# Yuming-Yang/FactorModeling

Measured on AMD Instinct MI355X. Metric: factor·asset·days/s (ops+IC+select), higher is better.
Workload: dtype f64

## Files before the change

factormodeling_amd/csrc/rank_ic.hip:

```cpp
#include "rank_fine.hpp"
#include "rank_launch.hpp"

namespace fmx {

__global__ void k_ic_empty(double* out, int64_t F, int64_t D, int L0, int L1, int NL) {
  const int64_t f = blockIdx.x;
  for (int m = 0; m < NL; ++m) {
    const int L = m == 0 ? L0 : L1;
    for (int64_t td = threadIdx.x; td < min<int64_t>(L, D); td += blockDim.x) {
      double* o = out + ((int64_t)(m * 4) * F + f) * D + td;
      o[0] = 0.0;
      o[F * D] = qnan();
      o[2 * F * D] = qnan();
      o[3 * F * D] = qnan();
    }
  }
}


fmx_status br_ic_daily(const double* X, const double* R, int64_t F, int64_t D, int64_t A, int64_t ld,
                       const int32_t* lags_host, int n_lags, double* out, hipStream_t st) {
  const int nt = A <= 4096 ? 512 : 1024;
  const size_t lds_fr = std::max<size_t>((size_t)(FRG<FR_K_IC>::NB + 1) * 8, (size_t)A * 13 + 16);
  auto fr_table = FMX_EMAX_TABLE(k_ic_daily_fr);
  const bool fine = rank_impl() == RANK_IMPL_FINE && lds_fits(fr_table(nt, br_emax(A, nt)), lds_fr);
  const size_t lds = fine ? lds_fr : (size_t)std::max<int64_t>(A, nt) * 8 + (size_t)((A + 15) & ~15ll);
  if (!fine && !lds_fits(FMX_EMAX_TABLE(k_ic_daily_br)(nt, br_emax(A, nt)), lds)) {
    set_error("row too long for the IC kernels' LDS (rank it once with fmx_cs_rank_winsor and use "
              "fmx_ic_daily_ranked)");
    return FMX_ERR_UNSUPPORTED;
  }
  for (int base = 0; base < n_lags; base += 2) {
    int NL = std::min(2, n_lags - base);
    int L0 = lags_host[base], L1 = NL > 1 ? lags_host[base + 1] : 0;
    double* o = out + (int64_t)base * 4 * F * D;
    k_ic_empty<<<(unsigned)F, 64, 0, st>>>(o, F, D, L0, L1, NL);
    FMX_LAUNCH_CHECK("k_ic_empty");
    void* args[] = {(void*)&X, (void*)&R, (void*)&F, (void*)&D, (void*)&A, (void*)&ld, (void*)&L0, (void*)&L1,
                    (void*)&NL, (void*)&o};
    fmx_status e = fine ? launch_br(fr_table, nt, A, F, D, lds, args, st)
                        : launch_br(FMX_EMAX_TABLE(k_ic_daily_br), nt, A, F, D, lds, args, st);
    if (e) return e;
  }
  return FMX_OK;
}

constexpr int ICW_PC = 256;
__global__ void __launch_bounds__(256)
k_nan_positions(const double* __restrict__ Rt, int64_t D, int64_t A, int64_t ld, int32_t* __restrict__ pos,
                int32_t* __restrict__ npos) {
  const int lane = threadIdx.x & 63;
  const int64_t d = (int64_t)blockIdx.x * 4 + (threadIdx.x >> 6);
  if (d >= D) return;
  const double* r = Rt + d * ld;
  const uint64_t lt = (1ull << lane) - 1ull;
  int c = 0;
  for (int64_t i0 = 0; i0 < A; i0 += 64) {
    const int64_t i = i0 + lane;
    const bool nan = i < A && !(r[i] == r[i]);
    const uint64_t b = __ballot(nan);
    const int at = c + __popcll(b & lt);
    if (nan && at < ICW_PC) pos[d * ICW_PC + at] = (int32_t)i;
    c += __popcll(b);
  }
  if (lane == 0) npos[d] = c;
}

constexpr int ICW_WAVES = 4;
#ifndef ICW_PF
#define ICW_PF 1
#endif
constexpr int ICW_EC = 256;
constexpr uint64_t ICW_NO_ENTRY = 0xffffffff00000000ull;

#ifndef ICW_MINW
#define ICW_MINW 6
#endif
__global__ void __launch_bounds__(64 * ICW_WAVES, ICW_MINW)
k_ic_wave(const double* __restrict__ X, const fmx_rank2_t* __restrict__ RK, const double* __restrict__ Rt, int64_t F,
          int64_t D, int64_t A, int64_t ld, int L0, int L1, int NL, double* __restrict__ out,
          const int32_t* __restrict__ pos, const int32_t* __restrict__ npos, int32_t* __restrict__ ovf) {
  extern __shared__ uint32_t icw_lds[];
  __shared__ double scr[ICW_WAVES * 32];
  const int lane = threadIdx.x & 63, wid = __builtin_amdgcn_readfirstlane((int)(threadIdx.x >> 6));
  const int64_t row = (int64_t)blockIdx.x * ICW_WAVES + wid;
  if (row >= F * D) return;
  const int64_t s = row / F, f = row % F;
  const int lagv[2] = {L0, L1};
  const double* rr[2];
  bool act[2];
#pragma unroll
  for (int m = 0; m < 2; ++m) {
    act[m] = m < NL && s + lagv[m] < D;
    rr[m] = Rt + (act[m] ? s + lagv[m] : s) * ld;
  }
  if (!act[0] && !act[1]) return;
  const double* xf = X + (f * D + s) * ld;
  const fmx_rank2_t* rkf = RK + (f * D + s) * ld;
  const int nb = (int)((2 * A) >> 6) + 1;
  const int nbp = (nb + 1) & ~1;
  uint32_t* T[2];
  uint64_t* T64[2];
  uint32_t* eb[2];
#pragma unroll
  for (int m = 0; m < 2; ++m) {
    T[m] = icw_lds + (wid * 2 + m) * (2 * nbp + ICW_EC);
    T64[m] = reinterpret_cast<uint64_t*>(T[m]);
    eb[m] = T[m] + 2 * nbp;
  }
  int ne[2] = {0, 0};
  bool over = false;
  uint32_t er[2][ICW_EC / 64];
  int es[2][ICW_EC / 64];
  const int An = (int)A;
  double xq[ICW_PF], rq[ICW_PF][2];
  uint32_t kq[ICW_PF];
  auto load = [&](int i0, int s) {
    const int i = i0 + lane;
    if (i0 + 64 <= An) {
      xq[s] = xf[i];
      kq[s] = (uint32_t)rkf[i];
#pragma unroll
      for (int m = 0; m < 2; ++m) rq[s][m] = rr[m][i];
    } else {
      const bool in = i < An;
      xq[s] = in ? xf[i] : qnan();
      kq[s] = in ? (uint32_t)rkf[i] : 0u;
#pragma unroll
      for (int m = 0; m < 2; ++m) rq[s][m] = in ? rr[m][i] : qnan();
    }
  };
#pragma unroll
  for (int s = 0; s < ICW_PF; ++s) load(64 * s, s);
#pragma unroll
  for (int m = 0; m < 2; ++m) {
    for (int b = lane; b < nbp; b += 64) T64[m][b] = 0ull;
#pragma unroll
    for (int q = 0; q < ICW_EC / 64; ++q) { er[m][q] = 0u; es[m][q] = 0; }
  }
  __builtin_amdgcn_wave_barrier();
  int cl[2];
#pragma unroll
  for (int m = 0; m < 2; ++m) cl[m] = act[m] ? npos[s + lagv[m]] : 0;
  over = cl[0] > ICW_PC || cl[1] > ICW_PC;
  if (!over) {
    const int cmax = cl[0] > cl[1] ? cl[0] : cl[1];
    const int32_t* pp[2] = {pos + (s + (act[0] ? lagv[0] : 0)) * ICW_PC, pos + (s + (act[1] ? lagv[1] : 0)) * ICW_PC};
#pragma unroll
    for (int q = 0; q < ICW_EC / 64; ++q) {
      if (64 * q >= cmax) break;
      const int j = 64 * q + lane;
      int p[2];
#pragma unroll
      for (int m = 0; m < 2; ++m) p[m] = pp[m][j];
#pragma unroll
      for (int m = 0; m < 2; ++m) p[m] = j < cl[m] ? p[m] : 0;
      uint32_t r2[2];
#pragma unroll
      for (int m = 0; m < 2; ++m) r2[m] = (uint32_t)rkf[p[m]];
#pragma unroll
      for (int m = 0; m < 2; ++m) {
        const uint32_t e = j < cl[m] ? r2[m] : 0u;
        er[m][q] = e;
        if (e) es[m][q] = (int)atomicAdd(&T[m][e >> 6], 1u);
        ne[m] += __popcll(__ballot(e != 0u));
      }
    }
  }
  if (over) {
    if (lane == 0) {
      const int q = atomicAdd(&ovf[0], 1);
      ovf[1 + q] = (int32_t)row;
    }
    return;
  }
  __builtin_amdgcn_wave_barrier();
#pragma unroll
  for (int m = 0; m < 2; ++m) {
    if (ne[m] == 0) continue;
    constexpr int RMAX = 9;
    const int R = (nbp + 63) >> 6;
    int cn[RMAX];
    int loc = 0;
#pragma unroll
    for (int q = 0; q < RMAX; ++q) {
      const int b = lane * R + q;
      cn[q] = (q < R && b < nbp) ? (int)T[m][b] : 0;
      loc += cn[q];
    }
    int incl = loc;
#pragma unroll
    for (int o = 1; o < 64; o <<= 1) {
      const int u = fr_up(incl, o, lane);
      if (lane >= o) incl += u;
    }
    int run = incl - loc;
    int st[RMAX];
    asm volatile("s_waitcnt lgkmcnt(0)" ::: "memory");
    __builtin_amdgcn_wave_barrier();
#pragma unroll
    for (int q = 0; q < RMAX; ++q) {
      const int b = lane * R + q;
      st[q] = run;
      if (q < R && b < nbp) T64[m][b] = ICW_NO_ENTRY | (uint64_t)((uint32_t)(2 * run) | ((uint32_t)cn[q] << 16));
      run += cn[q];
    }
    asm volatile("s_waitcnt lgkmcnt(0)" ::: "memory");
    __builtin_amdgcn_wave_barrier();
#pragma unroll
    for (int q = 0; q < ICW_EC / 64; ++q)
      if (er[m][q]) eb[m][(((uint32_t)T64[m][er[m][q] >> 6] & 0xffffu) >> 1) + es[m][q]] = er[m][q];
    asm volatile("s_waitcnt lgkmcnt(0)" ::: "memory");
    __builtin_amdgcn_wave_barrier();
#pragma unroll
    for (int q = 0; q < RMAX; ++q) {
      const int b = lane * R + q;
      if (q < R && b < nbp && cn[q] > 0) {
        const uint64_t e0 = eb[m][st[q]], e1 = cn[q] > 1 ? eb[m][st[q] + 1] : 0xffffu;
        T64[m][b] = (uint64_t)((uint32_t)(2 * st[q]) | ((uint32_t)cn[q] << 16)) | (e0 << 32) | (e1 << 48);
      }
    }
  }
#pragma unroll
  for (int m = 0; m < 2; ++m)
    if (ne[m] == 0)
      for (int b = lane; b < nbp; b += 64) T64[m][b] = ICW_NO_ENTRY;
  __builtin_amdgcn_wave_barrier();
  double sm[2][6];
  uint64_t kk[2] = {0, 0};
  double ax[2] = {0.0, 0.0}, ar[2] = {0.0, 0.0};
  bool ref[2] = {false, false};
  int cnt[2] = {0, 0};
  uint64_t dm[4] = {0, 0, 0, 0};
#pragma unroll
  for (int m = 0; m < 2; ++m)
#pragma unroll
    for (int q = 0; q < 6; ++q) sm[m][q] = 0.0;
  auto next = [&](int i0, double& x, uint32_t& rk, double (&r)[2]) {
    x = xq[0];
    rk = kq[0];
    r[0] = rq[0][0];
    r[1] = rq[0][1];
#pragma unroll
    for (int s = 0; s + 1 < ICW_PF; ++s) {
      xq[s] = xq[s + 1];
      kq[s] = kq[s + 1];
      rq[s][0] = rq[s + 1][0];
      rq[s][1] = rq[s + 1][1];
    }
    if (i0 + 64 * ICW_PF < An) load(i0 + 64 * ICW_PF, ICW_PF - 1);
  };
  auto pair_rank = [&](int m, uint32_t rk) {
    const uint64_t tb = T64[m][rk >> 6];
    const uint32_t lo = (uint32_t)tb, hi = (uint32_t)(tb >> 32);
    const uint32_t j0 = (lo & 0xffffu) >> 1, nj = lo >> 16, j1 = j0 + nj;
    const uint32_t e0 = hi & 0xffffu, e1 = hi >> 16;
    int corr = (int)(lo & 0xffffu) + (e0 < rk ? 1 : 0) + (e0 <= rk ? 1 : 0) + (e1 < rk ? 1 : 0) + (e1 <= rk ? 1 : 0);
    for (uint32_t j = j0 + 2; j < j1; ++j) {
      const uint32_t e = eb[m][j];
      corr += (e < rk ? 1 : 0) + (e <= rk ? 1 : 0);
    }
    return rk - (uint32_t)corr;
  };
  auto accum = [&](int m, bool p, uint64_t bp, double x, uint32_t k2, double r) {
    dm[2 * m] |= bp & __ballot(x != ax[m]);
    dm[2 * m + 1] |= bp & __ballot(r != ar[m]);
    if (!p) return;
    const double dx = x - ax[m], dy = r - ar[m];
    sm[m][0] += dx; sm[m][1] += dy;
    sm[m][2] = __builtin_fma(dx, dx, sm[m][2]);
    sm[m][3] = __builtin_fma(dy, dy, sm[m][3]);
    sm[m][4] = __builtin_fma(dx, dy, sm[m][4]);
    sm[m][5] = __builtin_fma((double)k2, dy, sm[m][5]);
    kk[m] += (uint64_t)k2 * k2;
  };
  ref[0] = !act[0];
  ref[1] = !act[1];
  int i0 = 0;
  for (; i0 < An && !(ref[0] && ref[1]); i0 += 64) {
    double x, r[2];
    uint32_t rk;
    next(i0, x, rk, r);
    const uint32_t k2[2] = {pair_rank(0, rk), pair_rank(1, rk)};
#pragma unroll
    for (int m = 0; m < 2; ++m) {
      const bool p = (x == x) & (r[m] == r[m]);
      const uint64_t bp = __ballot(p);
      cnt[m] += __popcll(bp);
      if (!ref[m] && bp) {
        const int l = __ffsll((unsigned long long)bp) - 1;
        ax[m] = fr_readlane_d(x, l);
        ar[m] = fr_readlane_d(r[m], l);
        ref[m] = true;
      }
      if (ref[m]) accum(m, p, bp, x, k2[m], r[m]);
    }
  }
  for (; i0 < An; i0 += 64) {
    double x, r[2];
    uint32_t rk;
    next(i0, x, rk, r);
    const uint32_t k2[2] = {pair_rank(0, rk), pair_rank(1, rk)};
    const bool xo = x == x;
#pragma unroll
    for (int m = 0; m < 2; ++m) {
      const bool p = xo & (r[m] == r[m]);
      const uint64_t bp = __ballot(p);
      cnt[m] += __popcll(bp);
      accum(m, p, bp, x, k2[m], r[m]);
    }
  }
  double* sc = scr + wid * 32;
  {
    double a[16];
#pragma unroll
    for (int q = 0; q < 6; ++q) { a[q] = sm[0][q]; a[6 + q] = sm[1][q]; }
    a[12] = (double)kk[0];
    a[13] = (double)kk[1];
    a[14] = a[15] = 0.0;
    fr_part_bfly<16, false>(a, scr, 32, 0);
  }
  uint32_t dflags = 0;
#pragma unroll
  for (int q = 0; q < 4; ++q) dflags |= (dm[q] != 0 ? 1u : 0u) << q;
  __builtin_amdgcn_wave_barrier();
  __builtin_amdgcn_fence(__ATOMIC_ACQUIRE, "wavefront");
  if (lane == 0) {
#pragma unroll
    for (int m = 0; m < 2; ++m) {
      if (!act[m]) continue;
      const int64_t td = s + lagv[m];
      double* o = out + ((int64_t)(m * 4) * F + f) * D + td;
      const int64_t stp = F * D;
      const double nn = (double)cnt[m];
      double ic = qnan(), ric = qnan(), beta = qnan();
      if (cnt[m] >= 3) {
        const double* w = sc + 6 * m;
        const double sx = w[0], sy = w[1];
        const bool fconst = !((dflags >> (2 * m)) & 1), rconst = !((dflags >> (2 * m + 1)) & 1);
        if (!fconst && !rconst) {
          const double sxy = w[4] - sx * sy / nn;
          const double sxx = w[2] - sx * sx / nn;
          const double syy = w[3] - sy * sy / nn;
          const double skk = sc[12 + m] / 4.0 - nn * (nn + 1.0) * (nn + 1.0) / 4.0;
          const double sky = 0.5 * w[5] - 0.5 * (nn + 1.0) * sy;
          ic = fmin(1.0, fmax(-1.0, sxy / sqrt(sxx * syy)));
          ric = fmin(1.0, fmax(-1.0, sky / sqrt(skk * syy)));
        }
        const double a = ax[m], b = ar[m];
        const double sxx_raw = w[2] + 2.0 * a * sx + nn * a * a;
        const double sxr_raw = w[4] + a * sy + b * sx + nn * a * b;
        beta = sxx_raw > 0 ? sxr_raw / sxx_raw : qnan();
      }
      o[0] = nn;
      o[stp] = ic;
      o[2 * stp] = ric;
      o[3 * stp] = beta;
    }
  }
}


int64_t ic_ranked_work_len(int64_t F, int64_t D) { return D * (ICW_PC + 1) + 1 + F * D; }

fmx_status br_ic_ranked(const double* X, const fmx_rank2_t* RK, const double* R, int64_t F, int64_t D, int64_t A,
                        int64_t ld, const int32_t* lags_host, int n_lags, double* out, int32_t* work, hipStream_t st) {
  const int nt = 1024;
  const void* kl = FMX_EMAX_TABLE(k_ic_ranked_list)(nt, br_emax(A, nt));
  if (!kl) { set_error("row too long for the ranked IC kernels (A > 16384)"); return FMX_ERR_UNSUPPORTED; }
  if (F * D > 0x7fffffffll) { set_error("too many rows for one launch"); return FMX_ERR_UNSUPPORTED; }
  int32_t* pos = work;
  int32_t* npos = work + D * ICW_PC;
  int32_t* ovf = npos + D;
  k_nan_positions<<<(unsigned)((D + 3) / 4), 256, 0, st>>>(R, D, A, ld, pos, npos);
  FMX_LAUNCH_CHECK("k_nan_positions");
  const int list_grid = 2 * device_cu_count();
  const unsigned wave_grid = (unsigned)((F * D + ICW_WAVES - 1) / ICW_WAVES);
  for (int base = 0; base < n_lags; base += 2) {
    int NL = std::min(2, n_lags - base);
    int L0 = lags_host[base], L1 = NL > 1 ? lags_host[base + 1] : 0;
    double* o = out + (int64_t)base * 4 * F * D;
    k_ic_empty<<<(unsigned)F, 64, 0, st>>>(o, F, D, L0, L1, NL);
    FMX_LAUNCH_CHECK("k_ic_empty");
    FMX_HIP(hipMemsetAsync(ovf, 0, sizeof(int32_t), st));
    const int nbp = ((int)((2 * A) >> 6) + 2) & ~1;
    const size_t lds = sizeof(uint32_t) * (ICW_WAVES * 2 * (size_t)(2 * nbp + ICW_EC) + 2);
    k_ic_wave<<<wave_grid, 64 * ICW_WAVES, lds, st>>>(X, RK, R, F, D, A, ld, L0, L1, NL, o, pos, npos, ovf);
    FMX_LAUNCH_CHECK("k_ic_wave");
    void* args[] = {(void*)&X, (void*)&RK, (void*)&R, (void*)&F, (void*)&D, (void*)&A, (void*)&ld, (void*)&L0,
                    (void*)&L1, (void*)&NL, (void*)&o, (void*)&ovf};
    const unsigned g = (unsigned)std::min<int64_t>(F * D, list_grid);
    FMX_HIP(hipLaunchKernel(kl, dim3(g), dim3(nt), args, 0, st));
  }
  return FMX_OK;
}


__global__ void __launch_bounds__(256)
k_nan_bits(const double* __restrict__ R, int64_t A, int64_t ld, int64_t nw, uint32_t* __restrict__ bits) {
  const int lane = threadIdx.x & 63;
  const int64_t i0 = ((int64_t)blockIdx.x * 4 + (threadIdx.x >> 6)) * 64;
  if (i0 >= nw * 32) return;
  const int64_t d = blockIdx.y, i = i0 + lane;
  const bool nan = i < A && !(R[d * ld + i] == R[d * ld + i]);
  const uint64_t b = __ballot(nan);
  if (lane == 0) {
    bits[d * nw + (i0 >> 5)] = (uint32_t)b;
    bits[d * nw + (i0 >> 5) + 1] = (uint32_t)(b >> 32);
  }
}

__global__ void __launch_bounds__(64)
k_ret_anchor(const double* __restrict__ R, int64_t A, int64_t ld, double* __restrict__ rsh) {
  const int lane = threadIdx.x;
  const double* r = R + (int64_t)blockIdx.x * ld;
  double v = 0.0;
  for (int64_t i0 = 0; i0 < A; i0 += 64) {
    const double x = i0 + lane < A ? r[i0 + lane] : qnan();
    const uint64_t b = __ballot(x == x);
    if (b) {
      v = fr_readlane_d(x, __ffsll((unsigned long long)b) - 1);
      break;
    }
  }
  if (lane == 0) rsh[blockIdx.x] = v;
}

static int64_t nanb_words(int64_t A) { return (A + 63) / 64 * 2; }

int64_t rank_ic_work_len(int64_t F, int64_t D, int64_t A) { return 2 * D + D * nanb_words(A) + 1 + F * D; }

template <int NT, int E> constexpr auto kcrwi = k_cs_rank_fa<NT, E, false, true, true>;
template <int NT, int E> constexpr auto kcri = k_cs_rank_fa<NT, E, false, false, true>;

fmx_status br_cs_rank_winsor_ic(const double* X, double* Yr, double* Yw, const double* R, int64_t F, int64_t D,
                                int64_t A, int64_t ld, double qlo, double qhi, const int32_t* lags, int n_lags,
                                fmx_rank2_t* RK, int32_t* work, double* out, hipStream_t st) {
  const int nt_fa = fa_nt(A);
  const size_t lds_fr = std::max<size_t>({(size_t)A * 8, (size_t)FR_CS_WORDS * 4, (size_t)fr_ic_lds_bytes(A, nt_fa)});
  const int E = br_emax(A, nt_fa);
  const void* k = E < 0 ? nullptr : (Yr ? FMX_EMAX_TABLE(kcrwi)(nt_fa, E) : FMX_EMAX_TABLE(kcri)(nt_fa, E));
  const void* kl = FMX_EMAX_TABLE(k_ic_ranked_list)(1024, br_emax(A, 1024));
  if (!k || !kl || !lds_fits(k, lds_fr)) {
    set_error("fmx_cs_rank_winsor_ic: rows of A <= 16384 assets");
    return FMX_ERR_UNSUPPORTED;
  }
  if (F * D > 0x7fffffffll) { set_error("too many rows for one launch"); return FMX_ERR_UNSUPPORTED; }
  const int64_t nw = nanb_words(A);
  double* rsh = reinterpret_cast<double*>(work);
  uint32_t* nanb = reinterpret_cast<uint32_t*>(work + 2 * D);
  int32_t* ovf = work + 2 * D + D * nw;
  k_nan_bits<<<dim3((unsigned)ceil_div(nw, 8), (unsigned)D), 256, 0, st>>>(R, A, ld, nw, nanb);
  FMX_LAUNCH_CHECK("k_nan_bits");
  k_ret_anchor<<<(unsigned)D, 64, 0, st>>>(R, A, ld, rsh);
  FMX_LAUNCH_CHECK("k_ret_anchor");
  int L0 = lags[0], L1 = n_lags > 1 ? lags[1] : 0, NL = n_lags;
  k_ic_empty<<<(unsigned)F, 64, 0, st>>>(out, F, D, L0, L1, NL);
  FMX_LAUNCH_CHECK("k_ic_empty");
  FMX_HIP(hipMemsetAsync(ovf, 0, sizeof(int32_t), st));
  FrIc ic{R, nanb, rsh, F, nw, L0, L1, NL, out, ovf, RK};
  FrZn zn{};
  int method = FMX_RANK_AVERAGE;
  const uint8_t* present = nullptr;
  fmx_rank2_t* RKrow = nullptr;
  const size_t loff = (size_t)fr_list_off(A, FR_CS_WORDS);
  const FrListLds ll = fr_list_lds(k, A, loff, lds_fr > loff ? lds_fr - loff : 0);
  int lcap = ll.cap;
  void* args[] = {(void*)&X, (void*)&Yr, (void*)&D, (void*)&A, (void*)&ld, (void*)&method, (void*)&present,
                  (void*)&Yw, (void*)&qlo, (void*)&qhi, (void*)&RKrow, (void*)&ic, (void*)&zn, (void*)&lcap};
  FMX_HIP(set_dyn_lds(k, ll.bytes));
  FMX_HIP(hipLaunchKernel(k, fmx_grid2(F, D), dim3(nt_fa), args, ll.bytes, st));
  const int list_grid = 2 * device_cu_count();
  const fmx_rank2_t* RKc = RK;
  void* largs[] = {(void*)&X, (void*)&RKc, (void*)&R, (void*)&F, (void*)&D, (void*)&A, (void*)&ld, (void*)&L0,
                   (void*)&L1, (void*)&NL, (void*)&out, (void*)&ovf};
  const unsigned g = (unsigned)std::min<int64_t>(F * D, list_grid);
  FMX_HIP(hipLaunchKernel(kl, dim3(g), dim3(1024), largs, 0, st));
  return FMX_OK;
}

}

BR_PHASE_EXPORT(fmx_debug_phase_ic)
```

Before: 45.73 billion.

## Interleave per-lag rank tables in LDS and fold empty-output and overflow reset into kernels

Interleaves the two per-lag bucket tables in LDS so one 128-bit LDS read fetches both lags' bucket entries for a rank. The long-chain correction loop now runs only when a ballot shows some lane needs it. The separate k_ic_empty kernel is replaced by having tail-row waves write the empty-IC values inline, and the first overflow-counter memset is folded into k_nan_positions. The change also adds an unguarded full-chunk load loop using byte-offset addressing, and switches the k² accumulation from integer to FMA in double. This cuts launches and LDS traffic, but the edge-write indexing and the interleaved layout add correctness risk.

```diff
diff --git a/factormodeling_amd/csrc/rank_ic.hip b/factormodeling_amd/csrc/rank_ic.hip
--- a/factormodeling_amd/csrc/rank_ic.hip
+++ b/factormodeling_amd/csrc/rank_ic.hip
@@ -48,8 +48,9 @@
 constexpr int ICW_PC = 256;
 __global__ void __launch_bounds__(256)
 k_nan_positions(const double* __restrict__ Rt, int64_t D, int64_t A, int64_t ld, int32_t* __restrict__ pos,
-                int32_t* __restrict__ npos) {
+                int32_t* __restrict__ npos, int32_t* __restrict__ ovf) {
   const int lane = threadIdx.x & 63;
+  if (blockIdx.x == 0 && threadIdx.x == 0) ovf[0] = 0;
   const int64_t d = (int64_t)blockIdx.x * 4 + (threadIdx.x >> 6);
   if (d >= D) return;
   const double* r = Rt + d * ld;
@@ -80,7 +81,7 @@
 k_ic_wave(const double* __restrict__ X, const fmx_rank2_t* __restrict__ RK, const double* __restrict__ Rt, int64_t F,
           int64_t D, int64_t A, int64_t ld, int L0, int L1, int NL, double* __restrict__ out,
           const int32_t* __restrict__ pos, const int32_t* __restrict__ npos, int32_t* __restrict__ ovf) {
-  extern __shared__ uint32_t icw_lds[];
+  extern __shared__ __attribute__((aligned(16))) uint32_t icw_lds[];
   __shared__ double scr[ICW_WAVES * 32];
   const int lane = threadIdx.x & 63, wid = __builtin_amdgcn_readfirstlane((int)(threadIdx.x >> 6));
   const int64_t row = (int64_t)blockIdx.x * ICW_WAVES + wid;
@@ -94,20 +95,22 @@
     act[m] = m < NL && s + lagv[m] < D;
     rr[m] = Rt + (act[m] ? s + lagv[m] : s) * ld;
   }
+  const int edge = __builtin_amdgcn_readfirstlane((NL > 0 && !act[0] ? 1 : 0) | (NL > 1 && !act[1] ? 2 : 0));
+  if (edge) {
+    const int m = lane >> 2, q = lane & 3;
+    if (lane < 8 && ((edge >> m) & 1)) {
+      const int64_t L = m ? L1 : L0, td = s - (D > L ? D - L : 0);
+      out[((int64_t)(m * 4 + q) * F + f) * D + td] = q == 0 ? 0.0 : qnan();
+    }
+  }
   if (!act[0] && !act[1]) return;
   const double* xf = X + (f * D + s) * ld;
   const fmx_rank2_t* rkf = RK + (f * D + s) * ld;
   const int nb = (int)((2 * A) >> 6) + 1;
   const int nbp = (nb + 1) & ~1;
-  uint32_t* T[2];
-  uint64_t* T64[2];
-  uint32_t* eb[2];
-#pragma unroll
-  for (int m = 0; m < 2; ++m) {
-    T[m] = icw_lds + (wid * 2 + m) * (2 * nbp + ICW_EC);
-    T64[m] = reinterpret_cast<uint64_t*>(T[m]);
-    eb[m] = T[m] + 2 * nbp;
-  }
+  uint32_t* T = icw_lds + wid * 2 * (2 * nbp + ICW_EC);
+  uint64_t* T64 = reinterpret_cast<uint64_t*>(T);
+  uint32_t* eb[2] = {T + 4 * nbp, T + 4 * nbp + ICW_EC};
   int ne[2] = {0, 0};
   bool over = false;
   uint32_t er[2][ICW_EC / 64];
@@ -115,13 +118,17 @@
   const int An = (int)A;
   double xq[ICW_PF], rq[ICW_PF][2];
   uint32_t kq[ICW_PF];
+  auto load_full = [&](int i0, int s) {
+    const uint32_t ob = 8u * (uint32_t)(i0 + lane);
+    xq[s] = *fr_at(xf, ob);
+    kq[s] = (uint32_t)*fr_at(rkf, ob >> 2);
+#pragma unroll
+    for (int m = 0; m < 2; ++m) rq[s][m] = *fr_at(rr[m], ob);
+  };
   auto load = [&](int i0, int s) {
     const int i = i0 + lane;
     if (i0 + 64 <= An) {
-      xq[s] = xf[i];
-      kq[s] = (uint32_t)rkf[i];
-#pragma unroll
-      for (int m = 0; m < 2; ++m) rq[s][m] = rr[m][i];
+      load_full(i0, s);
     } else {
       const bool in = i < An;
       xq[s] = in ? xf[i] : qnan();
@@ -134,10 +141,10 @@
   for (int s = 0; s < ICW_PF; ++s) load(64 * s, s);
 #pragma unroll
   for (int m = 0; m < 2; ++m) {
-    for (int b = lane; b < nbp; b += 64) T64[m][b] = 0ull;
 #pragma unroll
     for (int q = 0; q < ICW_EC / 64; ++q) { er[m][q] = 0u; es[m][q] = 0; }
   }
+  for (int b = lane; b < 2 * nbp; b += 64) T64[b] = 0ull;
   __builtin_amdgcn_wave_barrier();
   int cl[2];
 #pragma unroll
@@ -162,7 +169,7 @@
       for (int m = 0; m < 2; ++m) {
         const uint32_t e = j < cl[m] ? r2[m] : 0u;
         er[m][q] = e;
-        if (e) es[m][q] = (int)atomicAdd(&T[m][e >> 6], 1u);
+        if (e) es[m][q] = (int)atomicAdd(&T[4 * (e >> 6) + 2 * m], 1u);
         ne[m] += __popcll(__ballot(e != 0u));
       }
     }
@@ -185,7 +192,7 @@
 #pragma unroll
     for (int q = 0; q < RMAX; ++q) {
       const int b = lane * R + q;
-      cn[q] = (q < R && b < nbp) ? (int)T[m][b] : 0;
+      cn[q] = (q < R && b < nbp) ? (int)T[4 * b + 2 * m] : 0;
       loc += cn[q];
     }
     int incl = loc;
@@ -202,14 +209,14 @@
     for (int q = 0; q < RMAX; ++q) {
       const int b = lane * R + q;
       st[q] = run;
-      if (q < R && b < nbp) T64[m][b] = ICW_NO_ENTRY | (uint64_t)((uint32_t)(2 * run) | ((uint32_t)cn[q] << 16));
+      if (q < R && b < nbp) T64[2 * b + m] = ICW_NO_ENTRY | (uint64_t)((uint32_t)(2 * run) | ((uint32_t)cn[q] << 16));
       run += cn[q];
     }
     asm volatile("s_waitcnt lgkmcnt(0)" ::: "memory");
     __builtin_amdgcn_wave_barrier();
 #pragma unroll
     for (int q = 0; q < ICW_EC / 64; ++q)
-      if (er[m][q]) eb[m][(((uint32_t)T64[m][er[m][q] >> 6] & 0xffffu) >> 1) + es[m][q]] = er[m][q];
+      if (er[m][q]) eb[m][(((uint32_t)T64[2 * (er[m][q] >> 6) + m] & 0xffffu) >> 1) + es[m][q]] = er[m][q];
     asm volatile("s_waitcnt lgkmcnt(0)" ::: "memory");
     __builtin_amdgcn_wave_barrier();
 #pragma unroll
@@ -217,17 +224,17 @@
       const int b = lane * R + q;
       if (q < R && b < nbp && cn[q] > 0) {
         const uint64_t e0 = eb[m][st[q]], e1 = cn[q] > 1 ? eb[m][st[q] + 1] : 0xffffu;
-        T64[m][b] = (uint64_t)((uint32_t)(2 * st[q]) | ((uint32_t)cn[q] << 16)) | (e0 << 32) | (e1 << 48);
+        T64[2 * b + m] = (uint64_t)((uint32_t)(2 * st[q]) | ((uint32_t)cn[q] << 16)) | (e0 << 32) | (e1 << 48);
       }
     }
   }
 #pragma unroll
   for (int m = 0; m < 2; ++m)
     if (ne[m] == 0)
-      for (int b = lane; b < nbp; b += 64) T64[m][b] = ICW_NO_ENTRY;
+      for (int b = lane; b < nbp; b += 64) T64[2 * b + m] = ICW_NO_ENTRY;
   __builtin_amdgcn_wave_barrier();
   double sm[2][6];
-  uint64_t kk[2] = {0, 0};
+  double kk[2] = {0.0, 0.0};
   double ax[2] = {0.0, 0.0}, ar[2] = {0.0, 0.0};
   bool ref[2] = {false, false};
   int cnt[2] = {0, 0};
@@ -236,7 +243,7 @@
   for (int m = 0; m < 2; ++m)
 #pragma unroll
     for (int q = 0; q < 6; ++q) sm[m][q] = 0.0;
-  auto next = [&](int i0, double& x, uint32_t& rk, double (&r)[2]) {
+  auto take = [&](double& x, uint32_t& rk, double (&r)[2]) {
     x = xq[0];
     rk = kq[0];
     r[0] = rq[0][0];
@@ -248,40 +255,65 @@
       rq[s][0] = rq[s + 1][0];
       rq[s][1] = rq[s + 1][1];
     }
+  };
+  auto next = [&](int i0, double& x, uint32_t& rk, double (&r)[2]) {
+    take(x, rk, r);
     if (i0 + 64 * ICW_PF < An) load(i0 + 64 * ICW_PF, ICW_PF - 1);
   };
-  auto pair_rank = [&](int m, uint32_t rk) {
-    const uint64_t tb = T64[m][rk >> 6];
-    const uint32_t lo = (uint32_t)tb, hi = (uint32_t)(tb >> 32);
-    const uint32_t j0 = (lo & 0xffffu) >> 1, nj = lo >> 16, j1 = j0 + nj;
-    const uint32_t e0 = hi & 0xffffu, e1 = hi >> 16;
-    int corr = (int)(lo & 0xffffu) + (e0 < rk ? 1 : 0) + (e0 <= rk ? 1 : 0) + (e1 < rk ? 1 : 0) + (e1 <= rk ? 1 : 0);
-    for (uint32_t j = j0 + 2; j < j1; ++j) {
-      const uint32_t e = eb[m][j];
-      corr += (e < rk ? 1 : 0) + (e <= rk ? 1 : 0);
-    }
-    return rk - (uint32_t)corr;
+  auto pair_ranks = [&](uint32_t rk, uint32_t (&k2)[2]) {
+    const uint4 tw = *reinterpret_cast<const uint4*>(T64 + 2 * (rk >> 6));
+    const uint32_t lo[2] = {tw.x, tw.z}, hi[2] = {tw.y, tw.w};
+    int corr[2];
+#pragma unroll
+    for (int m = 0; m < 2; ++m) {
+      const uint32_t e0 = hi[m] & 0xffffu, e1 = hi[m] >> 16;
+      corr[m] = (int)(lo[m] & 0xffffu) + (e0 < rk ? 1 : 0) + (e0 <= rk ? 1 : 0) + (e1 < rk ? 1 : 0) + (e1 <= rk ? 1 : 0);
+    }
+    if (__ballot(max(lo[0], lo[1]) >= (3u << 16))) {
+#pragma unroll
+      for (int m = 0; m < 2; ++m) {
+        const uint32_t j0 = (lo[m] & 0xffffu) >> 1, j1 = j0 + (lo[m] >> 16);
+        for (uint32_t j = j0 + 2; j < j1; ++j) {
+          const uint32_t e = eb[m][j];
+          corr[m] += (e < rk ? 1 : 0) + (e <= rk ? 1 : 0);
+        }
+      }
+    }
+#pragma unroll
+    for (int m = 0; m < 2; ++m) k2[m] = rk - (uint32_t)corr[m];
   };
   auto accum = [&](int m, bool p, uint64_t bp, double x, uint32_t k2, double r) {
     dm[2 * m] |= bp & __ballot(x != ax[m]);
     dm[2 * m + 1] |= bp & __ballot(r != ar[m]);
     if (!p) return;
-    const double dx = x - ax[m], dy = r - ar[m];
+    const double dx = x - ax[m], dy = r - ar[m], kd = (double)k2;
     sm[m][0] += dx; sm[m][1] += dy;
     sm[m][2] = __builtin_fma(dx, dx, sm[m][2]);
     sm[m][3] = __builtin_fma(dy, dy, sm[m][3]);
     sm[m][4] = __builtin_fma(dx, dy, sm[m][4]);
-    sm[m][5] = __builtin_fma((double)k2, dy, sm[m][5]);
-    kk[m] += (uint64_t)k2 * k2;
+    sm[m][5] = __builtin_fma(kd, dy, sm[m][5]);
+    kk[m] = __builtin_fma(kd, kd, kk[m]);
+  };
+  auto reduce = [&](double x, uint32_t rk, const double (&r)[2]) {
+    uint32_t k2[2];
+    pair_ranks(rk, k2);
+    const bool xo = x == x;
+#pragma unroll
+    for (int m = 0; m < 2; ++m) {
+      const bool p = xo & (r[m] == r[m]);
+      const uint64_t bp = __ballot(p);
+      cnt[m] += __popcll(bp);
+      accum(m, p, bp, x, k2[m], r[m]);
+    }
   };
   ref[0] = !act[0];
   ref[1] = !act[1];
   int i0 = 0;
   for (; i0 < An && !(ref[0] && ref[1]); i0 += 64) {
     double x, r[2];
-    uint32_t rk;
+    uint32_t rk, k2[2];
     next(i0, x, rk, r);
-    const uint32_t k2[2] = {pair_rank(0, rk), pair_rank(1, rk)};
+    pair_ranks(rk, k2);
 #pragma unroll
     for (int m = 0; m < 2; ++m) {
       const bool p = (x == x) & (r[m] == r[m]);
@@ -296,27 +328,26 @@
       if (ref[m]) accum(m, p, bp, x, k2[m], r[m]);
     }
   }
+  for (; i0 + 64 * (ICW_PF + 1) <= An; i0 += 64) {
+    double x, r[2];
+    uint32_t rk;
+    take(x, rk, r);
+    load_full(i0 + 64 * ICW_PF, ICW_PF - 1);
+    reduce(x, rk, r);
+  }
   for (; i0 < An; i0 += 64) {
     double x, r[2];
     uint32_t rk;
     next(i0, x, rk, r);
-    const uint32_t k2[2] = {pair_rank(0, rk), pair_rank(1, rk)};
-    const bool xo = x == x;
-#pragma unroll
-    for (int m = 0; m < 2; ++m) {
-      const bool p = xo & (r[m] == r[m]);
-      const uint64_t bp = __ballot(p);
-      cnt[m] += __popcll(bp);
-      accum(m, p, bp, x, k2[m], r[m]);
-    }
+    reduce(x, rk, r);
   }
   double* sc = scr + wid * 32;
   {
     double a[16];
 #pragma unroll
     for (int q = 0; q < 6; ++q) { a[q] = sm[0][q]; a[6 + q] = sm[1][q]; }
-    a[12] = (double)kk[0];
-    a[13] = (double)kk[1];
+    a[12] = kk[0];
+    a[13] = kk[1];
     a[14] = a[15] = 0.0;
     fr_part_bfly<16, false>(a, scr, 32, 0);
   }
@@ -372,7 +403,7 @@
   int32_t* pos = work;
   int32_t* npos = work + D * ICW_PC;
   int32_t* ovf = npos + D;
-  k_nan_positions<<<(unsigned)((D + 3) / 4), 256, 0, st>>>(R, D, A, ld, pos, npos);
+  k_nan_positions<<<(unsigned)((D + 3) / 4), 256, 0, st>>>(R, D, A, ld, pos, npos, ovf);
   FMX_LAUNCH_CHECK("k_nan_positions");
   const int list_grid = 2 * device_cu_count();
   const unsigned wave_grid = (unsigned)((F * D + ICW_WAVES - 1) / ICW_WAVES);
@@ -380,9 +411,7 @@
     int NL = std::min(2, n_lags - base);
     int L0 = lags_host[base], L1 = NL > 1 ? lags_host[base + 1] : 0;
     double* o = out + (int64_t)base * 4 * F * D;
-    k_ic_empty<<<(unsigned)F, 64, 0, st>>>(o, F, D, L0, L1, NL);
-    FMX_LAUNCH_CHECK("k_ic_empty");
-    FMX_HIP(hipMemsetAsync(ovf, 0, sizeof(int32_t), st));
+    if (base > 0) FMX_HIP(hipMemsetAsync(ovf, 0, sizeof(int32_t), st));
     const int nbp = ((int)((2 * A) >> 6) + 2) & ~1;
     const size_t lds = sizeof(uint32_t) * (ICW_WAVES * 2 * (size_t)(2 * nbp + ICW_EC) + 2);
     k_ic_wave<<<wave_grid, 64 * ICW_WAVES, lds, st>>>(X, RK, R, F, D, A, ld, L0, L1, NL, o, pos, npos, ovf);
```

New measurement: 45.73 billion. About the same (-0.0%).
